# imuncle/TSCM_Calib

Hardware: AMD Instinct MI355X
Metric: LM iterations/sec at 4 cams x 10k views (joint intrinsics+extrinsics, fp64) (higher is better)
Workload: dtype f64; 1 GPU; BASELINE config 4: 4 cams x 10000 views/cam, 20000 frames, 2160000 corners (9x6 board, sigma=0.1 px, seed 20244); parallelism=frames sharded over 1 GPU(s)

## Files before the change

include/tscm/tscm.h:

```cpp
#ifndef TSCM_H
#define TSCM_H

#include <stddef.h>

#ifdef __cplusplus
extern "C" {
#endif

#define TSCM_ABI_VERSION 6

enum {
    TSCM_OK = 0,
    TSCM_E_INVALID = -1,
    TSCM_E_NO_DEVICE = -2,
    TSCM_E_HIP = -3,
    TSCM_E_RCCL = -4,
    TSCM_E_UNSUPPORTED = -5,
    TSCM_E_NOMEM = -6,
    TSCM_E_PEER = -7
};

enum { TSCM_CONVERGENCE = 0, TSCM_NO_CONVERGENCE = 1, TSCM_FAILURE = 2 };

#define TSCM_MAX_ITERATIONS 255
// ... 76 lines not shown
    double seconds_solve;
    double seconds_total;
    double rmse;
} tscm_summary;

typedef struct tscm_solver tscm_solver;
typedef struct tscm_comm tscm_comm;

int tscm_abi_version(void);
const char *tscm_last_error(void);
int tscm_device_count(void);
int tscm_device_synchronize(int device);
int tscm_device_peak_fp64(int device, double *mfma_tflops, double *valu_tflops);
int tscm_device_peak_fp64_ex(int device, double peaks[3]);
int tscm_device_peak_fp32_mfma(int device, double *tflops);

void tscm_default_options(tscm_options *opt, int mono);

int tscm_solver_create(const tscm_problem *problem, int device, tscm_solver **out);
int tscm_solver_set_comm(tscm_solver *s, tscm_comm *comm);
int tscm_solver_debug_withhold_handoff(tscm_solver *s, int on);
int tscm_solver_debug_schur_rot(tscm_solver *s, int rot);
int tscm_solver_debug_reduced_backsub(tscm_solver *s, int on);
int tscm_solver_reruns(const tscm_solver *s);
int tscm_solver_solve(tscm_solver *s, const tscm_options *opt, tscm_summary *summary);
int tscm_solver_upload_params(tscm_solver *s, const double *cam_rt, const double *intr, const double *board_rt);
int tscm_solver_solve_resident(tscm_solver *s, const tscm_options *opt, tscm_summary *summary, int reset);
int tscm_solver_download_params(tscm_solver *s, double *cam_rt, double *intr, double *board_rt);
void tscm_solver_destroy(tscm_solver *s);
int tscm_solver_kernel_time(tscm_solver *s, int enable, int *launches, double *total_ms);
int tscm_solver_exchange_time(tscm_solver *s, int *n_T, double *ms_T, int *n_H, double *ms_H);

int tscm_solve_multi(const tscm_problem *problem, const tscm_options *opt, tscm_summary *summary);
int tscm_solve_mono(const tscm_problem *problem, const tscm_options *opt, tscm_summary *summary);

int tscm_eval_functor(const tscm_problem *problem, int device, double *residuals,
                      double *J_cam, double *J_board, double *J_intr, double *cost);

int tscm_eval_normal_equations(const tscm_problem *problem, int device, double *board_gram,
                               double *board_grad, double *view_cross, double *cam_gram,
                               double *cam_grad, double *cost);

int tscm_eval_normal_equations_ex(const tscm_problem *problem, int device, const tscm_options *opt,
                                  double *board_gram, double *board_grad, double *view_cross,
                                  double *cam_gram, double *cam_grad, double *cost);

// ... 540 lines not shown
```

tscm_calib_amd/api.py:

```python
from __future__ import annotations

import ctypes as C

import numpy as np

from . import lib as _l
from .problem import Problem


class Solver:

    def __init__(self, problem: Problem, device: int = 0, rank: int = 0, world: int = 1, *, weights=None, priors=None):
        self.problem = problem.normalised() if not _is_normalised(problem) else problem
        self.problem.validate()
        self._built, w = _l.corner_weights(self.problem, weights)
        self._cp = _l.c_problem(self._built)
        self._h = C.c_void_p()
        self.rank, self.world = rank, world
        _l.check(_l.lib().tscm_solver_create_sharded(C.byref(self._cp), device, rank, world, C.byref(self._h)))
        self._comm = None
        if w is not None:
            _l.check(_l.lib().tscm_solver_set_corner_weights(self._h, _l.dptr(w)))
        if priors is not None:
            self.set_camera_priors(priors)
# ... 23 lines not shown
        if weights is None:
            _l.check(_l.lib().tscm_solver_set_corner_weights(self._h, None))
            return
        _, w = _l.corner_weights(self.problem, weights, self._built.view_count)
        _l.check(_l.lib().tscm_solver_set_corner_weights(self._h, _l.dptr(w)))

    def set_fixed_intrinsics(self, fixed):
        w = _l.fixed_masks(fixed, self.problem.n_cameras)
        _l.check(_l.lib().tscm_solver_set_fixed_intrinsics(self._h, _l.ushort_ptr(w)))

    def set_camera_priors(self, priors):
        ptr, keep = _l.priors_ptr(priors, self.problem.n_cameras)
        _l.check(_l.lib().tscm_solver_set_camera_priors(self._h, ptr))
        del keep

    def debug_withhold_handoff(self, on=True):
        _l.check(_l.lib().tscm_solver_debug_withhold_handoff(self._h, int(on)))

    def debug_schur_rot(self, rot=0):
        _l.check(_l.lib().tscm_solver_debug_schur_rot(self._h, int(rot)))

    def debug_reduced_backsub(self, on=True):
        _l.check(_l.lib().tscm_solver_debug_reduced_backsub(self._h, int(bool(on))))

    def reruns(self) -> int:
        n = _l.lib().tscm_solver_reruns(self._h)
        if n < 0:
            _l.check(n)
        return n

    def solve(self, **options) -> dict:
        o = _l.default_options(self.problem.mono, **options)
        s = _l.CSummary()
        _l.check(_l.lib().tscm_solver_solve(self._h, C.byref(o), C.byref(s)))
        return _l.summary_dict(s)

    def upload_params(self, cam_rt=None, intr=None, board_rt=None):
        p = self.problem
        cam_rt = p.cam_rt if cam_rt is None else np.ascontiguousarray(cam_rt, dtype=np.float64)
        intr = p.intr if intr is None else np.ascontiguousarray(intr, dtype=np.float64)
        board_rt = p.board_rt if board_rt is None else np.ascontiguousarray(board_rt, dtype=np.float64)
        _l.check(_l.lib().tscm_solver_upload_params(self._h, _l.dptr(cam_rt), _l.dptr(intr), _l.dptr(board_rt)))

    def solve_resident(self, reset: bool = True, **options) -> dict:
        o = _l.default_options(self.problem.mono, **options)
        s = _l.CSummary()
# ... 109 lines not shown
    def solve_resident(self, reset: bool = True, **options) -> "list[dict]":
        o = _l.default_options(self.problem.mono, **options)
        hs = (C.c_void_p * self.world)(*[s._h for s in self.solvers])
        sums = (_l.CSummary * self.world)()
        _l.check(_l.lib().tscm_solver_solve_group(hs, self.world, C.byref(o), sums, 1 if reset else 0))
        return [_l.summary_dict(sums[r]) for r in range(self.world)]

    def close(self):
        for s in self.solvers:
            s.close()
        for c in self.comms:
            c.close()
        self.solvers, self.comms = [], []

    def __enter__(self):
        return self

    def __exit__(self, *a):
        self.close()


def debug_reduced_backsub_default(on=True):
    _l.check(_l.lib().tscm_solver_debug_reduced_backsub(None, int(bool(on))))


def _is_normalised(p: Problem) -> bool:
    ok = lambda a, dt: isinstance(a, np.ndarray) and a.dtype == dt and a.flags["C_CONTIGUOUS"]
    return (all(ok(getattr(p, n), np.float64) for n in ("board_xy", "obs_u", "obs_v", "cam_rt", "intr", "board_rt"))
            and all(ok(getattr(p, n), np.int32) for n in ("view_camera", "view_board", "view_offset", "view_count"))
            and ok(p.cam_pose_constant, np.uint8)
            and (p.board_pose_constant is None or ok(p.board_pose_constant, np.uint8)))


def camera_priors(problem: Problem, intr_sigma=None, cam_rt_sigma=None, mean=None, pixel_sigma: float = 1.0) -> "_l.CameraPriors":
    Cn = problem.n_cameras
    mean = mean or {}

    def weights(sig, per):
        s = np.broadcast_to(np.asarray(sig, dtype=np.float64), (Cn, per)).copy()
        if np.any(s < 0.0):
            raise ValueError("a prior's sigma must not be negative")
        w = np.zeros((Cn, per))
        ok = np.isfinite(s) & (s > 0.0)
        w[ok] = (float(pixel_sigma) / s[ok]) ** 2
        return w

# ... 488 lines not shown
```

tscm_calib_amd/csrc/tscm_columns.h:

```cpp
#ifndef TSCM_COLUMNS_H
#define TSCM_COLUMNS_H

#include "tscm_layout.h"
#include "tscm_nd_plan.h"
#include "tscm_exec_plan.h"

#include <algorithm>
#include <string>
#include <utility>
#include <vector>

namespace tscm {

constexpr int kColFree = 13;
constexpr int kColGrad = 13;

struct SolveTile { bool mine, rhsrow; int ri, cj; };
template <int TS, int G>
inline SolveTile solve_tile(int tid, int NP)
{
    constexpr int NT = (G * G + 63) / 64 * 64;
    auto owns = [&](int t) { const int ti = t / G, tj = t % G; return tj <= ti && ti < NP; };
    SolveTile t;
    t.mine = owns(tid); t.rhsrow = false;
// ... 10 lines not shown
constexpr int kMapOne = 1 << 30;
constexpr int kSolveMapThreads = 256;

constexpr int kExtNone = 0, kExtRow = 3, kExtSol = 4;
constexpr int kSolveExtPanels = 12;
TSCM_LAYOUT_FN bool solve_tile_live(int kind, int ri, int cj, int from, int tk)
{
    if (kind == kExtNone || !(ri > tk && cj >= tk && tk >= from)) return false;
    if (ri == cj && ri == tk + 1) return false;
    return !(kind == kExtRow && cj == tk);
}

struct ColumnPlan {
    std::vector<unsigned char> col_active;
    std::vector<unsigned char> col_ctl;
    std::vector<int> act_map;
    int n_act = 0;
    int cam_pre[9] = {};
    unsigned short cam_free[8] = {};
    std::vector<Int4> solve_map;
    std::vector<Int4> solve_ext;
    bool ext_fallback = false;
    int wave_sum_old = 0, wave_sum_new = 0;
    bool has_nd = false;
    NdPlan nd[2];
};

inline std::vector<Int4> plan_solve_map(const Layout &L, const ColumnPlan &c)
{
    constexpr int TS = 4, G = 16, NT = kSolveMapThreads;
    static_assert(NT == (G * G + 63) / 64 * 64, "one map entry per thread of k_solve_reduced<4, 16>");
    const int NP = (c.n_act + TS - 1) / TS;
    auto cmap = [&](int ci) { return ci < c.n_act ? c.act_map[ci] : -1; };
    auto t_offset = [&](int i, int j) {
        int lo = i >> 4, hi = j >> 4, a = i & 15, b = j & 15;
        if (lo > hi) { std::swap(lo, hi); std::swap(a, b); }
        const int bit = lo * 8 + hi;
        const unsigned long long m = L.pair_mask;
        return ((m >> bit) & 1ull) ? 256 * __builtin_popcountll(m & ((1ull << bit) - 1ull)) + a * 16 + b : -1;
    };
    std::vector<Int4> map((size_t)(kSolveMapSlots / 4) * NT);
    for (int tid = 0; tid < NT; ++tid) {
        const SolveTile tl = solve_tile<TS, G>(tid, NP);
        int off[kSolveMapSlots];
        std::fill(off, off + kSolveMapSlots, -1);
        off[kMapTile] = tl.ri; off[kMapTile + 1] = tl.cj; off[kMapTile + 2] = tl.mine ? 1 : tl.rhsrow ? 2 : 0;
// ... 46 lines not shown
    for (int i = 0; i < NP; ++i) {
        for (int j = i; j < NP; ++j) tiles.push_back(Tile{ kExtRow, NP + 1 + i, j, i, i, j - 1 });
        tiles.push_back(Tile{ kExtSol, NP + 1 + i, NP, i, i, NP - 1 });
    }
    std::stable_sort(tiles.begin(), tiles.end(), [](const Tile &a, const Tile &b) { return a.last != b.last ? a.last > b.last : a.first < b.first; });
    size_t room = 0;
    for (const auto &f : free_tid) room += f.size();
    if (room < tiles.size()) { c.ext_fallback = true; return; }
    std::vector<size_t> used(NW, 0);
    for (const Tile &t : tiles) {
        int best = -1, best_add = 0, best_base = 0;
        for (int w = 0; w < NW - 1; ++w) {
            if (used[w] == free_tid[w].size()) continue;
            int add = 0, base = 0;
            for (int tk = 0; tk < NP; ++tk) { add += tk >= t.first && tk <= t.last && !live[w][tk]; base += live[w][tk]; }
            if (best < 0 || add < best_add || (add == best_add && base > best_base)) { best = w; best_add = add; best_base = base; }
        }
        c.solve_ext[(size_t)free_tid[best][used[best]++]] = Int4{ t.kind, t.ri, t.cj, t.i };
        for (int tk = t.first; tk <= t.last; ++tk) live[best][tk] = 1;
    }
    c.wave_sum_new = wave_sum();
}

inline int plan_columns(const Layout &L, int C, const unsigned short *fixed, ColumnPlan &out, std::string &err)
{
    ColumnPlan c;
    const int n_pad = 16 * C;
    c.col_active.assign((size_t)n_pad, 0); c.col_ctl.assign((size_t)16 * kMaxCam, 0);
    std::vector<unsigned short> word(C, 0);
    for (int i = 0; i < n_pad; ++i) {
        const int m = i >> 4, a = i & 15;
        const bool act = L.cam_active[m] != 0, cst = L.cam_const[m] != 0;
        const unsigned f = fixed ? fixed[m] : 0u;
        const bool held = a >= 6 && a < kColFree && ((f >> (a - 6)) & 1u);
        const bool block_const = (f & TSCM_FIX_INTRINSICS) == TSCM_FIX_INTRINSICS;
        c.col_active[i] = (a < kColFree && act && !(a < 6 && cst) && !held) ? 1 : 0;
        const bool in_x = a < 6 ? (act && !cst) : a < 15 ? (act && !block_const) : false;
        c.col_ctl[i] = (unsigned char)((in_x ? 1 : 0) | (c.col_active[i] ? 2 : 0));
        if (c.col_active[i]) word[m] |= (unsigned short)(1u << a);
    }
    c.act_map.assign((size_t)n_pad, -1);
    for (int i = 0; i < n_pad; ++i) if (c.col_active[i]) c.act_map[c.n_act++] = i;
    std::fill(c.cam_pre, c.cam_pre + 9, c.n_act);
    if (C <= kMaxCamLds) {
        int run = 0;
        for (int m = 0; m < C; ++m) { c.cam_pre[m] = run; c.cam_free[m] = word[m]; run += __builtin_popcount(word[m]); }
    }
    if (C <= kDense4Cams) { c.solve_map = plan_solve_map(L, c); plan_solve_ext(c); }
    if (C <= kMaxCamLds && c.n_act > 0) {
        int ncols[kMaxCamLds];
        std::vector<int> cols((size_t)16 * C, -1);
        for (int m = 0; m < C; ++m) {
            ncols[m] = 0;
            for (int a = 0; a < 16; ++a) if ((word[m] >> a) & 1u) cols[16 * (size_t)m + ncols[m]++] = 16 * m + a;
        }
        if (!nd_build_plans_cols(C, ncols, cols.data(), L.pair_present.data(), L.bid_of.data(), c.nd))
            return layout_fail(err, TSCM_E_UNSUPPORTED, "internal error: the reduced system does not fit the register/LDS solver");
        const std::vector<int> want(c.act_map.begin(), c.act_map.begin() + c.n_act);
        for (const NdPlan &pl : c.nd) {
            std::vector<int> pc;
            for (int col : pl.pcol) if (col >= 0) pc.push_back(col);
            std::sort(pc.begin(), pc.end());
            if (pc != want) return layout_fail(err, TSCM_E_UNSUPPORTED, "internal error: elimination plan does not cover the free columns");
        }
        c.has_nd = true;
    }
    out = std::move(c);
    return 0;
}

}
// ... 3 lines not shown
```

tscm_calib_amd/csrc/tscm_solve_dense4.h:

```cpp
#pragma once

__device__ __forceinline__ double load_T_small(const DevProblem &P, const double *T, int i, int j)
{
    int lo = i >> 4, hi = j >> 4, a = i & 15, b = j & 15;
    if (lo > hi) { const int t = lo; lo = hi; hi = t; const int u = a; a = b; b = u; }
    const int bit = lo * 8 + hi;
    const unsigned long long m = P.pair_mask;
    const int tile = __popcll(m & ((1ull << bit) - 1ull));
    return ((m >> bit) & 1ull) ? T[256 * tile + a * 16 + b] : 0.0;
}

__host__ __device__ __forceinline__ int kth_set_bit16(unsigned w, int k)
{
    int pos = 0, c;
    c = __builtin_popcount(w & 0xffu); if (k >= c) { k -= c; w >>= 8; pos += 8; }
    c = __builtin_popcount(w & 0xfu);  if (k >= c) { k -= c; w >>= 4; pos += 4; }
    c = __builtin_popcount(w & 0x3u);  if (k >= c) { k -= c; w >>= 2; pos += 2; }
    c = (int)(w & 1u);                 if (k >= c) pos += 1;
    return pos;
}
__device__ __forceinline__ int compact_to_padded(const DevProblem &P, int ci)
{
    int base = 0, q0 = 0;
    unsigned w = P.cam_free[0];
// ... 182 lines not shown
        }
    };
    auto load_tile = [&](const double *src, double (&t)[TS][TS]) {
#pragma unroll
        for (int r = 0; r < TS; ++r)
#pragma unroll
            for (int c = 0; c < TS; ++c) t[r][c] = src[r * TS + c];
    };
    auto panel_solve = [&](const double (&At)[TS][TS], const PanelFactor &f, double (&x)[TS][TS]) {
#pragma unroll
        for (int r = 0; r < TS; ++r)
#pragma unroll
            for (int c = 0; c < TS; ++c) {
                double v = At[r][c];
#pragma unroll
                for (int q = 0; q < c; ++q) v -= x[r][q] * f.l[c][q];
                x[r][c] = v * f.il[c];
            }
    };
    __shared__ __attribute__((aligned(16))) double s_dt[2][TS * TS];
    const bool dthread = tid == NT - 1;
    if (cj == 0 && ri > 0 && pub) publish_tile(lds + xo, a);
    if (ri == 1 && cj == 1 && mine) publish_tile(s_dt[0], a);
    if (tid == 0 && NP > 0) factor_diag(a, 0);
    __syncthreads();
    for (int tk = 0; tk < NP; ++tk) {
        const double *Ar = Xb + (tk & 1) * (G * XT);
#ifdef TSCM_PHASE_PROFILE
        __shared__ long long s_ph[8];
        if (tk == 3 && (dthread || tid == 11 * G + 5)) s_ph[dthread ? 0 : 4] = wall_clock64();
#endif
        if (dthread && tk + 1 < NP) {
            PanelFactor f;
            double araw[TS][TS], dt[TS][TS], x[TS][TS], t[TS][TS];
            load_factor(f, tk);
            load_tile(Ar + (tk + 1) * XT, araw);
            load_tile(s_dt[tk & 1], dt);
            __builtin_amdgcn_sched_barrier(0);
            panel_solve(araw, f, x);
#pragma unroll
            for (int r = 0; r < TS; ++r)
#pragma unroll
                for (int c = 0; c <= r; ++c) {
                    double v = dt[r][c];
#pragma unroll
                    for (int q = 0; q < TS; ++q) v -= x[r][q] * x[c][q];
                    t[r][c] = v;
                }
#ifdef TSCM_PHASE_PROFILE
            if (tk == 3) { asm volatile("" : "+v"(t[3][3])); s_ph[1] = wall_clock64(); }
#endif
            factor_diag(t, tk + 1);
#ifdef TSCM_PHASE_PROFILE
// ... 16 lines not shown
                if (rhsrow) {
#pragma unroll
                    for (int c = 0; c < TS; ++c) wp[tk * TS + c] = xi[0][c];
                }
            } else {
                double xj[TS][TS];
                panel_solve(aj, f, xj);
#pragma unroll
                for (int r = 0; r < TS; ++r)
#pragma unroll
                    for (int c = 0; c < TS; ++c) {
                        double v = a[r][c];
#pragma unroll
                        for (int q = 0; q < TS; ++q) v -= xi[r][q] * xj[c][q];
                        a[r][c] = v;
                    }
            }
        }
        {
            const bool col = cj == tk + 1 && ri > tk + 1 && pub, dg = ri == tk + 2 && cj == tk + 2 && mine;
            if (col || dg) publish_tile(col ? lds + xo + ((tk + 1) & 1) * xs : s_dt[(tk + 1) & 1], a);
        }
#ifdef TSCM_PHASE_PROFILE
        if (tk == 3 && tid == 11 * G + 5) { asm volatile("" : "+v"(a[3][3])); s_ph[5] = wall_clock64(); }
        if (tk + 1 < NP) __syncthreads();
        if (tk == 3 && tid == 0) { s_ph[6] = wall_clock64(); printf("  panel 3: D x,t %lld  factor %lld | update %lld | to barrier exit %lld\n", s_ph[1] - s_ph[0], s_ph[2] - s_ph[1], s_ph[5] - s_ph[4], s_ph[6] - s_ph[0]); }
#else
        if (tk + 1 < NP) __syncthreads();
#endif
    }
    if (stile) {
#pragma unroll
        for (int r = 0; r < TS; ++r) { const int pc = s_c2p[from * TS + r]; if (pc >= 0) yv[pc] = -a[r][0]; }
    }
    if (!ext_on && cj < ri && mine) {
#pragma unroll
        for (int r = 0; r < TS; ++r)
#pragma unroll
            for (int c = 0; c < TS; ++c) Lm[(ri * TS + r) * LD + cj * TS + c] = a[r][c];
    }
    __syncthreads();
    PHASE_STAMP(ts2);
#ifdef TSCM_PHASE_PROFILE
    const long long cy2 = clock64();
#endif
    TailOperands tail_ops = {};
    if (!ext_on) tail_prefetch(P, S, cur, H, tail_ops);
// ... 54 lines not shown
```

tscm_calib_amd/csrc/tscm_solver.hip:

```cpp
#include "tscm/tscm.h"
#include "tscm_host.h"
#include "tscm_kernels.h"
#include "tscm_launch_seq.h"
#include "tscm_mono_batch.h"

#include <hip/hip_runtime.h>
#include <hip/hip_ext.h>
#include <rccl/rccl.h>

#include <algorithm>
#include <atomic>
#include <chrono>
#include <cstdio>
#include <cstdlib>
#include <cmath>
#include <cstring>
#include <memory>
#include <numeric>
#include <string>
#include <thread>
#include <vector>

using namespace tscm;

// ... 95 lines not shown
    NdPlan plan[2];
    const int4 *d_nd_map[2] = { nullptr, nullptr };
    const int *d_nd_tab[2] = { nullptr, nullptr }, *d_nd_bs[2] = { nullptr, nullptr };
    size_t lds_nd[2] = { 0, 0 }, lds_dense4 = 0;
    size_t lds_eval4 = 0;
    EvalKernel eval[kEvalFamilies] = {};
    LossArg loss{};
    bool weighted = false;
    double *d_obs_w = nullptr;
    std::vector<double> h_obs_u, h_obs_v;
    std::vector<int> p_view_count;
    double w_sum = 0.0;
    long n_kept = 0;
    std::vector<double> pr_cam_mean, pr_cam_w, pr_intr_mean, pr_intr_w;
    std::vector<unsigned char> col_free;
    double *d_prior = nullptr;
    int n_priors = 0;
    PriorArg prior_arg() const { return PriorArg{ d_prior, d_prior + 16 * (size_t)C }; }
    std::vector<unsigned short> fixed;
    int n_cu = 1;
    int schur_rot = 0;
    bool ext_planned = false;
    bool force_backsub = false;
    double *d_view_sq = nullptr;
    int timing = 0;
    unsigned ev_count[3] = { 0, 0, 0 };
    std::vector<std::pair<hipEvent_t, hipEvent_t>> ev;
    std::vector<int> ev_kind;
    size_t ev_used = 0;
    int t_launches[3] = { 0, 0, 0 };
    double t_ms[3] = { 0.0, 0.0, 0.0 };
};

struct SolverDelete { void operator()(tscm_solver *s) const { tscm_solver_destroy(s); } };
using SolverPtr = std::unique_ptr<tscm_solver, SolverDelete>;

static int create_scoped(const tscm_problem *p, int device, SolverPtr &sp)
{
    tscm_solver *s = nullptr;
    if (int rc = tscm_solver_create(p, device, &s)) return rc;
    sp.reset(s);
    return 0;
}

extern "C" int tscm_abi_version(void) { return TSCM_ABI_VERSION; }
extern "C" const char *tscm_last_error(void) { return g_err.c_str(); }
// ... 124 lines not shown
{
    if (!s) return fail(TSCM_E_INVALID, "solver is NULL");
    if (int rc = check_camera_priors(priors, s->C)) return rc;
    if (priors && s->world > 1) return fail(TSCM_E_UNSUPPORTED, "camera priors on a sharded solver (world > 1) are not supported");
    auto keep = [&](std::vector<double> &dst, const double *src, int per) { if (priors && src) dst.assign(src, src + per * (size_t)s->C); else dst.clear(); };
    keep(s->pr_cam_mean, priors ? priors->cam_rt_mean : nullptr, 6); keep(s->pr_cam_w, priors ? priors->cam_rt_weight : nullptr, 6);
    keep(s->pr_intr_mean, priors ? priors->intr_mean : nullptr, 9); keep(s->pr_intr_w, priors ? priors->intr_weight : nullptr, 9);
    return refresh_priors(s);
}

extern "C" void tscm_solver_destroy(tscm_solver *s)
{
    if (!s) return;
    (void)hipSetDevice(s->device);
    s->stream = s->own_stream;
    if (s->stream) (void)hipStreamSynchronize(s->stream);
    for (auto &e : s->ev) { (void)hipEventDestroy(e.first); (void)hipEventDestroy(e.second); }
    if (s->h_ctrl) (void)hipHostFree(s->h_ctrl);
    if (s->stream) (void)hipStreamDestroy(s->stream);
    delete s;
}

static std::atomic<bool> g_force_backsub{ false };

static int apply_columns(tscm_solver *s, const ColumnPlan &c)
{
    DevProblem &P = s->P;
    HIP_TRY(hipSetDevice(s->device));
    HIP_TRY(hipStreamSynchronize(s->stream));
    HIP_TRY(hipMemcpy(const_cast<unsigned char *>(P.col_active), c.col_active.data(), c.col_active.size(), hipMemcpyHostToDevice));
    HIP_TRY(hipMemcpy(const_cast<unsigned char *>(P.col_ctl), c.col_ctl.data(), c.col_ctl.size(), hipMemcpyHostToDevice));
    HIP_TRY(hipMemcpy(const_cast<int *>(P.act_map), c.act_map.data(), sizeof(int) * c.act_map.size(), hipMemcpyHostToDevice));
    P.n_act = c.n_act;
    std::copy(std::begin(c.cam_pre), std::end(c.cam_pre), P.cam_pre);
    std::copy(std::begin(c.cam_free), std::end(c.cam_free), P.cam_free);
    static_assert(sizeof(Int4) == sizeof(int4), "the operand map is uploaded as it is");
    if (!c.solve_map.empty()) {
        HIP_TRY(hipMemcpy(const_cast<int4 *>(P.solve_map), c.solve_map.data(), sizeof(Int4) * c.solve_map.size(), hipMemcpyHostToDevice));
        HIP_TRY(hipMemcpy(const_cast<int4 *>(P.solve_ext), c.solve_ext.data(), sizeof(Int4) * c.solve_ext.size(), hipMemcpyHostToDevice));
        s->ext_planned = !c.ext_fallback;
        P.solve_ext_on = s->ext_planned && !s->force_backsub;
    }
    if (c.has_nd) {
        for (int v = 0; v < 2; ++v) {
            const NdPlan &pl = c.nd[v];
            s->mem.release(s->d_nd_map[v]); s->mem.release(s->d_nd_tab[v]); s->mem.release(s->d_nd_bs[v]);
            s->d_nd_map[v] = nullptr; s->d_nd_tab[v] = nullptr; s->d_nd_bs[v] = nullptr;
            HIP_TRY(s->mem.upload(&s->d_nd_map[v], reinterpret_cast<const int4 *>(pl.map.data()), pl.map.size() / 4));
            HIP_TRY(s->mem.upload(&s->d_nd_tab[v], pl.tab));
            HIP_TRY(s->mem.upload(&s->d_nd_bs[v], pl.bs_tab));
            s->lds_nd[v] = sizeof(double) * pl.lds_doubles;
            s->plan[v] = pl;
        }
        {
            const size_t lds_max = std::max(std::max(s->lds_nd[0], s->lds_nd[1]), s->lds_bs);
            if (lds_max > 64 * 1024)
                for (const void *k : { reinterpret_cast<const void *>(k_solve_nd<1, true>), reinterpret_cast<const void *>(k_solve_nd<2, true>),
                                       reinterpret_cast<const void *>(k_solve_nd<1, false>), reinterpret_cast<const void *>(k_solve_nd<2, false>) })
                    HIP_TRY(hipFuncSetAttribute(k, hipFuncAttributeMaxDynamicSharedMemorySize, (int)lds_max));
        }
        for (int v = 0; v < 2; ++v) {
            const size_t lds = std::max(s->lds_nd[v], s->lds_bs);
            int per_cu = 0;
            if (s->plan[v].tpt == 1) HIP_TRY(hipOccupancyMaxActiveBlocksPerMultiprocessor(&per_cu, reinterpret_cast<const void *>(k_solve_nd<1, true>), kNdThreads, lds));
// ... 149 lines not shown
    for (int *flag : { S.t_count, S.y_flag, S.fac_fail }) HIP_TRY(hipMemset(flag, 0, sizeof(int)));
    for (int k = 0; k < 2; ++k) if (V) HIP_TRY(hipMemset(S.rec[k], 0, sizeof(double) * (size_t)kRec * V));
    HIP_TRY(hipMemset(S.stats_count, 0, 256)); HIP_TRY(hipMemset(S.stats_flag, 0, 256));
    HIP_TRY(hipMemset(S.ctl_pub, 0, sizeof(CtlPub)));
    HIP_TRY(hipMemset(S.T, 0, sizeof(double) * 256 * (size_t)L.n_bids));
    HIP_TRY(hipMemset(S.H_stage, 0, sizeof(double) * (256 * (size_t)C + kScal + world)));
    HIP_TRY(hipMemset(S.campart2, 0, sizeof(double) * 512 * (size_t)C));
    HIP_TRY(hipMemset(S.ctrl, 0, sizeof(Ctrl)));
    HIP_TRY(hipMemset(S.ctrl_snap, 0, sizeof(CtrlHead)));
    HIP_TRY(hipHostMalloc(reinterpret_cast<void **>(&s->h_ctrl), sizeof(Ctrl)));
    HIP_TRY(hipHostGetDevicePointer(reinterpret_cast<void **>(&s->d_h_ctrl), s->h_ctrl, 0));

    s->lds_eval = 4 * lds_eval_bytes;
    s->lds_eval32 = sizeof(double) * (size_t)eval_f32_lds_doubles(p->n_points, g4.ks);
    s->lds_eval4 = lds_eval4;
    if (s->lds_eval32 > 64 * 1024)
        for (int f = F32; f < kEvalFamilies; ++f) HIP_TRY(hipFuncSetAttribute(reinterpret_cast<const void *>(s->eval[f]), hipFuncAttributeMaxDynamicSharedMemorySize, (int)s->lds_eval32));
    ColumnPlan cols;
    {
        std::string err;
        if (int rc = plan_columns(L, C, nullptr, cols, err)) return fail(rc, err);
    }
    if (C <= kDense4Cams) {
        int4 *map = nullptr;
        HIP_TRY(s->mem.alloc(&map, (size_t)(kSolveMapSlots / 4) * kSolveMapThreads));
        P.solve_map = map;
        int4 *ext = nullptr;
        HIP_TRY(s->mem.alloc(&ext, (size_t)kSolveMapThreads));
        P.solve_ext = ext;
        s->force_backsub = g_force_backsub.load();
        const size_t NN = 64, TT = 4, NPD = 64;
        s->lds_dense4 = sizeof(double) * (NN * (NN + 2) + 2 * (NN / TT) * (TT * TT + 2) + 2 * NN + 3 * NPD);
        int per_cu = 0;
        HIP_TRY(hipOccupancyMaxActiveBlocksPerMultiprocessor(&per_cu, reinterpret_cast<const void *>(k_solve_reduced<4, 16, 64, true>), 256, std::max(s->lds_dense4, s->lds_bs)));
        s->dev.dense4_resident = per_cu * prop.multiProcessorCount;
    }
    if (C > kMaxCamLds) {
        const int NN = (cols.n_act + 15) & ~15;
        const size_t lds_max = solve_big_lds_bytes(NN, s->n_pad);
        HIP_TRY(s->mem.alloc(&S.Abig, (size_t)256 * (NN / 16 + 1) * (NN / 16 + 2) / 2));
        if (lds_max > 64 * 1024) HIP_TRY(hipFuncSetAttribute(reinterpret_cast<const void *>(k_solve_reduced_big), hipFuncAttributeMaxDynamicSharedMemorySize, (int)lds_max));
    }
    if (int rc = apply_columns(s, cols)) return rc;
    if (s->lds_eval > 160 * 1024) return fail(TSCM_E_UNSUPPORTED, "board has too many corners for the LDS board-point tile");
    HIP_TRY(hipDeviceSynchronize());
    *out = sp.release();
    return 0;
}

extern "C" int tscm_solver_create(const tscm_problem *p, int device, tscm_solver **out)
{
    return tscm_solver_create_sharded(p, device, 0, 1, out);
}
// ... 1 lines not shown
static CommKind comm_kind(const tscm_comm *c) { return !c ? kCommNone : c->world > 1 || c->group ? kCommShared : kCommOneRank; }

extern "C" int tscm_solver_debug_withhold_handoff(tscm_solver *s, int on)
{
    if (!s) return fail(TSCM_E_INVALID, "solver is NULL");
    s->withhold_next = on == 3 ? kWithholdStats : on ? kWithholdProducer : 0;
    s->no_rerun_next = on == 2;
    return 0;
}

extern "C" int tscm_solver_debug_schur_rot(tscm_solver *s, int rot)
{
    if (!s) return fail(TSCM_E_INVALID, "solver is NULL");
    if (rot != 0 && rot != 2) return fail(TSCM_E_INVALID, "rot must be 0 or 2");
    s->schur_rot = rot;
    return 0;
}

extern "C" int tscm_solver_debug_reduced_backsub(tscm_solver *s, int on)
{
    if (on != 0 && on != 1) return fail(TSCM_E_INVALID, "on must be 0 or 1");
    if (!s) { g_force_backsub.store(on != 0); return 0; }
    s->force_backsub = on != 0;
    s->P.solve_ext_on = s->ext_planned && !s->force_backsub;
    return 0;
}

extern "C" int tscm_solver_reruns(const tscm_solver *s)
{
    if (!s) return fail(TSCM_E_INVALID, "solver is NULL");
    return s->n_reruns;
}

extern "C" int tscm_solver_set_comm(tscm_solver *s, tscm_comm *comm)
{
    if (!s) return fail(TSCM_E_INVALID, "solver is NULL");
    if (comm && comm->device != s->device) return fail(TSCM_E_INVALID, "communicator and solver live on different devices");
    if (comm && (comm->world != s->world || comm->rank != s->rank))
        return fail(TSCM_E_INVALID, "communicator rank / world differ from the solver's shard (tscm_solver_create_sharded)");
    s->comm_reg = comm;
    s->comm = uses_comm(comm_kind(comm), 0) ? comm : nullptr;
    return 0;
}

extern "C" int tscm_solver_upload_params(tscm_solver *s, const double *cam_rt, const double *intr, const double *board_rt)
{
    if (!s || !intr || (!board_rt && s->L.B_total)) return fail(TSCM_E_INVALID, "NULL argument");
// ... 191 lines not shown
    }
    double *buf = t_buffer ? s0->S.T : s0->S.H_stage;
    if (int rc = timed_begin(s0, t_buffer ? 1 : 2, s0->stream, &e1)) return rc;
    if (int rc = comm_allreduce(s0->comm, buf, n, s0->stream)) return rc;
    if (e1) HIP_TRY(hipEventRecord(e1, s0->stream));
    return 0;
}

static int enqueue(tscm_solver *s, const Launch &l)
{
    const DevProblem &P = s->P;
    const DevState &S = s->S;
    hipStream_t st = s->stream;
    const dim3 grid(l.grid);
    auto schur = [&](auto kernel) { hipLaunchKernelGGL(kernel, grid, dim3(256), 0, st, P, S, l.chunk0, l.ctl, l.first_round, l.ce, l.target, l.n_chunks, s->schur_rot); };
    auto nd = [&](auto kernel) {
        const int v = l.nd;
        hipLaunchKernelGGL(kernel, grid, dim3(kNdThreads), std::max(s->lds_nd[v], l.n_bs ? s->lds_bs : (size_t)0), st, P, S, s->d_nd_map[v], s->d_nd_tab[v], s->d_nd_bs[v],
                           s->plan[v].dims(), l.epoch, l.withhold, l.n_prod, l.n_bs, l.f32);
    };
    const size_t lds_dense4 = std::max(s->lds_dense4, l.n_bs ? s->lds_bs : (size_t)0);
    auto dense4 = [&](auto kernel) {
        DevProblem Pd = P;
        if (s->xp.f32()) Pd.solve_ext_on = 0;
        hipLaunchKernelGGL(kernel, grid, dim3(256), lds_dense4, st, Pd, S, l.epoch, l.withhold, l.n_prod, l.n_bs, l.f32);
    };
    switch (l.k) {
    case Kern::BeginViewPrep: {
        const bool init = l.start == Start::Init, bak = l.start == Start::Backup;
        hipLaunchKernelGGL(k_begin_view_prep, grid, dim3(kVPrepThreads), 0, st, P, S, s->head,
                           init ? s->d_init_cam : bak ? s->d_start_cam : nullptr, init ? s->d_init_intr : bak ? s->d_start_intr : nullptr,
                           init ? s->d_init_board : bak ? s->d_start_board : nullptr,
                           bak ? nullptr : s->d_start_cam, bak ? nullptr : s->d_start_intr, bak ? nullptr : s->d_start_board, l.f32);
        break;
    }
    case Kern::Eval: return launch_eval(s, l.cand);
    case Kern::ReduceControl: hipLaunchKernelGGL(k_reduce_control, grid, dim3(256), 0, st, P, S, l.cand, l.init, l.have_backsub); break;
    case Kern::ReduceStats:
        if (s->xp.priors) hipLaunchKernelGGL(k_reduce_stats_prior, grid, dim3(256), 0, st, P, S, l.cand, l.init, s->prior_arg());
        else hipLaunchKernelGGL(k_reduce_stats, grid, dim3(256), 0, st, P, S, l.cand, l.init);
        break;
    case Kern::FinalizeEval: hipLaunchKernelGGL(k_finalize_eval, grid, dim3(256), 0, st, P, S, l.have_backsub); break;
    case Kern::Control: hipLaunchKernelGGL(k_control, grid, dim3(256), 0, st, P, S, l.init); break;
    case Kern::SchurFactor: hipLaunchKernelGGL(k_schur_factor, grid, dim3(256), 0, st, P, S); break;
    case Kern::Schur1: schur(k_schur_gram<1>); break;
    case Kern::Schur2: schur(k_schur_gram<2>); break;
    case Kern::Schur3: schur(k_schur_gram<3>); break;
// ... 1104 lines not shown
```

tscm_calib_amd/lib.py:

```python
from __future__ import annotations

import ctypes as C
import os
import subprocess

import numpy as np

_HERE = os.path.dirname(os.path.abspath(__file__))
CSRC = os.path.join(_HERE, "csrc")
LIB_PATH = os.path.join(CSRC, "libtscm_hip.so")
UNIQUE_ID_BYTES = 128
IPC_HANDLE_BYTES = 80
MAX_ITERATIONS = 255
EXEC_SEPARATE_T_REDUCE = 1
EXEC_KEEP_SINGLE_RANK_COMM = 2
EXEC_GRAM_16X16 = 4
EXEC_SEPARATE_BACKSUB = 8
EXEC_SEPARATE_CONTROL = 16
EXEC_DENSE_REDUCED_ORDER = 32
EXEC_GRAPH_REDUCED_ORDER = 64
EXEC_SEPARATE_STATS = 128
LOSS_NONE, LOSS_HUBER, LOSS_SOFT_L1, LOSS_CAUCHY = 0, 1, 2, 3
LOSS_KINDS = {None: LOSS_NONE, "none": LOSS_NONE, "huber": LOSS_HUBER, "soft_l1": LOSS_SOFT_L1, "cauchy": LOSS_CAUCHY}
PROJ_PERSPECTIVE, PROJ_LONGLAT, PROJ_CYLINDRICAL, PROJ_STEREOGRAPHIC, PROJ_EQUIRECT = 0, 1, 2, 3, 4
# ... 153 lines not shown
    _fields_ = [("camera_a", C.c_int), ("camera_b", C.c_int), ("board_rt", C.c_double * 6)]


class CResidualParams(C.Structure):
    _fields_ = [("struct_size", C.c_int), ("loss_kind", C.c_int), ("loss_scale", C.c_double), ("grid_w", C.c_int), ("grid_h", C.c_int),
                ("image_width", C.c_int), ("image_height", C.c_int), ("n_angle_bins", C.c_int), ("pad", C.c_int), ("max_angle", C.c_double),
                ("clamp", C.c_double)]


class CResidualInfo(C.Structure):
    _fields_ = [("struct_size", C.c_int), ("n_views_used", C.c_int), ("n_used", C.c_longlong), ("sum_w", C.c_double), ("cost", C.c_double),
                ("rmse", C.c_double), ("grid_outside", C.c_longlong * 32), ("angle_outside", C.c_longlong * 32), ("seconds_kernel", C.c_double * 4)]


class CCornerSet(C.Structure):
    _fields_ = [
        ("n_cameras", C.c_int), ("n_boards", C.c_int), ("board_cols", C.c_int), ("board_rows", C.c_int), ("pitch", C.c_double),
        ("image_width", C.c_int), ("image_height", C.c_int), ("has", C.c_void_p), ("pix_u", C.c_void_p), ("pix_v", C.c_void_p),
    ]


EXPORTS = [
    "tscm_abi_version", "tscm_last_error", "tscm_device_count", "tscm_device_synchronize", "tscm_device_peak_fp64", "tscm_device_peak_fp64_ex", "tscm_device_peak_fp32_mfma", "tscm_default_options",
    "tscm_solver_create", "tscm_solver_set_comm", "tscm_solver_debug_withhold_handoff", "tscm_solver_debug_schur_rot", "tscm_solver_debug_reduced_backsub", "tscm_solver_reruns", "tscm_solver_solve", "tscm_solver_upload_params",
    "tscm_solver_solve_resident", "tscm_solver_download_params", "tscm_solver_destroy",
    "tscm_solver_kernel_time", "tscm_solver_exchange_time", "tscm_solve_multi", "tscm_solve_mono", "tscm_eval_functor",
    "tscm_eval_normal_equations", "tscm_eval_normal_equations_ex", "tscm_eval_step_ex", "tscm_project_points", "tscm_unproject_pixels",
    "tscm_reprojection_error", "tscm_comm_unique_id", "tscm_comm_create", "tscm_comm_destroy",
    "tscm_shard_frames", "tscm_solver_create_sharded", "tscm_comm_create_local", "tscm_comm_ipc_open", "tscm_comm_ipc_connect", "tscm_solver_solve_group",
    "tscm_solver_gather_boards", "tscm_comm_info", "tscm_rig_init", "tscm_rig_stage_errors", "tscm_yaml_format", "tscm_yaml_write", "tscm_yaml_parse",
    "tscm_yaml_read", "tscm_build_maps", "tscm_estimate_focal", "tscm_poses_from_r1r2t",
    "tscm_estimate_extrinsic", "tscm_estimate_focal_rows", "tscm_estimate_extrinsic_stages", "tscm_corners_write", "tscm_corners_read", "tscm_corners_free",
    "tscm_detect_corners", "tscm_detect_corners_batch", "tscm_corner_planes_batch", "tscm_corner_candidates_free", "tscm_chessboards_from_corners", "tscm_chessboards_free", "tscm_remap",
    "tscm_solver_set_loss", "tscm_solve_robust", "tscm_eval_normal_equations_robust", "tscm_eval_step_robust",
    "tscm_solver_eval_normal_equations",
    "tscm_solver_set_fixed_intrinsics", "tscm_solve_fixed", "tscm_eval_step_fixed", "tscm_solve_mono_batch",
    "tscm_covariance", "tscm_covariance_from_normal_equations",
    "tscm_solver_set_corner_weights", "tscm_solve_weighted", "tscm_eval_normal_equations_weighted", "tscm_eval_step_weighted",
    "tscm_solve_mono_batch_weighted", "tscm_covariance_weighted",
    "tscm_solver_set_camera_priors", "tscm_solve_prior", "tscm_eval_normal_equations_prior", "tscm_eval_step_prior", "tscm_covariance_prior",
    "tscm_projection_uncertainty", "tscm_projection_uncertainty_seconds",
    "tscm_view_gain", "tscm_view_gain_apply", "tscm_view_gain_seconds",
    "tscm_residual_default_params", "tscm_residual_report", "tscm_residual_debug_chunk_target",
    "tscm_build_maps_ex", "tscm_rectify_points",
    "tscm_stereo_default_params", "tscm_stereo_match", "tscm_stereo_stages", "tscm_stereo_stage_times", "tscm_stereo_points",
    "tscm_stereo_filter_default_params", "tscm_stereo_filter", "tscm_stereo_filter_stages",
    "tscm_stereo_fill_default_params", "tscm_stereo_fill", "tscm_stereo_fill_stages",
# ... 30 lines not shown
    L = C.CDLL(LIB_PATH)
    dp, ip, vp = C.POINTER(C.c_double), C.POINTER(C.c_int), C.c_void_p
    L.tscm_abi_version.restype = C.c_int
    L.tscm_last_error.restype = C.c_char_p
    L.tscm_device_count.restype = C.c_int
    L.tscm_device_synchronize.argtypes = [C.c_int]
    L.tscm_device_peak_fp64.argtypes = [C.c_int, dp, dp]
    L.tscm_device_peak_fp64_ex.argtypes = [C.c_int, dp]
    L.tscm_device_peak_fp32_mfma.argtypes = [C.c_int, dp]
    L.tscm_default_options.argtypes = [C.POINTER(COptions), C.c_int]
    L.tscm_default_options.restype = None
    L.tscm_solver_create.argtypes = [C.POINTER(CProblem), C.c_int, C.POINTER(vp)]
    L.tscm_solver_create_sharded.argtypes = [C.POINTER(CProblem), C.c_int, C.c_int, C.c_int, C.POINTER(vp)]
    L.tscm_comm_create_local.argtypes = [C.c_int, C.c_int, C.POINTER(vp)]
    L.tscm_comm_ipc_open.argtypes = [C.c_int, C.c_int, C.c_int, C.c_size_t, C.POINTER(vp), C.POINTER(C.c_ubyte)]
    L.tscm_comm_ipc_connect.argtypes = [vp, C.POINTER(C.c_ubyte)]
    L.tscm_solver_solve_group.argtypes = [C.POINTER(vp), C.c_int, C.POINTER(COptions), C.POINTER(CSummary), C.c_int]
    L.tscm_solver_gather_boards.argtypes = [vp, dp]
    L.tscm_comm_info.argtypes = [vp, ip, ip, ip]
    L.tscm_solver_set_comm.argtypes = [vp, vp]
    L.tscm_solver_debug_withhold_handoff.argtypes = [vp, C.c_int]
    L.tscm_solver_debug_schur_rot.argtypes = [vp, C.c_int]
    L.tscm_solver_debug_reduced_backsub.argtypes = [vp, C.c_int]
    L.tscm_solver_reruns.argtypes = [vp]
    L.tscm_solver_solve.argtypes = [vp, C.POINTER(COptions), C.POINTER(CSummary)]
    L.tscm_solver_upload_params.argtypes = [vp, dp, dp, dp]
    L.tscm_solver_solve_resident.argtypes = [vp, C.POINTER(COptions), C.POINTER(CSummary), C.c_int]
    L.tscm_solver_download_params.argtypes = [vp, dp, dp, dp]
    L.tscm_solver_destroy.argtypes = [vp]
    L.tscm_solver_destroy.restype = None
    L.tscm_solver_kernel_time.argtypes = [vp, C.c_int, ip, dp]
    L.tscm_solver_exchange_time.argtypes = [vp, ip, dp, ip, dp]
    L.tscm_solve_multi.argtypes = [C.POINTER(CProblem), C.POINTER(COptions), C.POINTER(CSummary)]
    L.tscm_solve_mono.argtypes = [C.POINTER(CProblem), C.POINTER(COptions), C.POINTER(CSummary)]
    L.tscm_eval_functor.argtypes = [C.POINTER(CProblem), C.c_int, dp, dp, dp, dp, dp]
    L.tscm_eval_normal_equations.argtypes = [C.POINTER(CProblem), C.c_int, dp, dp, dp, dp, dp, dp]
    L.tscm_eval_normal_equations_ex.argtypes = [C.POINTER(CProblem), C.c_int, C.POINTER(COptions), dp, dp, dp, dp, dp, dp]
    L.tscm_eval_step_ex.argtypes = [C.POINTER(CProblem), C.c_int, C.POINTER(COptions), dp, dp, dp, ip, C.POINTER(CSummary)]
    L.tscm_solver_set_loss.argtypes = [vp, C.c_int, C.c_double]
    L.tscm_solve_robust.argtypes = [C.POINTER(CProblem), C.POINTER(COptions), C.c_int, C.c_double, C.POINTER(CSummary)]
    L.tscm_eval_normal_equations_robust.argtypes = [C.POINTER(CProblem), C.c_int, C.POINTER(COptions), C.c_int, C.c_double, dp, dp, dp, dp, dp, dp]
    L.tscm_eval_step_robust.argtypes = [C.POINTER(CProblem), C.c_int, C.POINTER(COptions), C.c_int, C.c_double, dp, dp, dp, ip, C.POINTER(CSummary)]
    L.tscm_solver_eval_normal_equations.argtypes = [vp, C.POINTER(COptions), C.c_int, dp, dp, dp, dp, dp, dp]
    usp = C.POINTER(C.c_ushort)
    L.tscm_solver_set_fixed_intrinsics.argtypes = [vp, usp]
    L.tscm_solve_fixed.argtypes = [C.POINTER(CProblem), C.POINTER(COptions), usp, C.c_int, C.c_double, C.POINTER(CSummary)]
# ... 309 lines not shown
```

Before: 9469 LM iterations/s.

## Reseat dense Schur solve tiles onto threads to retire waves early

Adds a host-side planner that permutes which thread owns each tile in the dense 4-camera Schur factorization. Tiles are grouped into wavefronts by the last panel in which they are live, so whole waves go idle sooner. The remapped operand tables are uploaded in two variants, one for the extended path and one for backsub or f32. The kernel now picks the diagonal-factor thread by tile ownership instead of thread id 0. The plan is kept only when it lowers the count of active waves summed over panels, and it adds extra device tables plus a debug toggle.

```diff
diff --git a/include/tscm/tscm.h b/include/tscm/tscm.h
--- a/include/tscm/tscm.h
+++ b/include/tscm/tscm.h
@@ -122,6 +122,8 @@
 int tscm_solver_debug_withhold_handoff(tscm_solver *s, int on);
 int tscm_solver_debug_schur_rot(tscm_solver *s, int rot);
 int tscm_solver_debug_reduced_backsub(tscm_solver *s, int on);
+int tscm_solver_debug_solve_seating(tscm_solver *s, int on);
+int tscm_solver_solve_seating_info(const tscm_solver *s, int *info);
 int tscm_solver_reruns(const tscm_solver *s);
 int tscm_solver_solve(tscm_solver *s, const tscm_options *opt, tscm_summary *summary);
 int tscm_solver_upload_params(tscm_solver *s, const double *cam_rt, const double *intr, const double *board_rt);
diff --git a/tscm_calib_amd/api.py b/tscm_calib_amd/api.py
--- a/tscm_calib_amd/api.py
+++ b/tscm_calib_amd/api.py
@@ -69,6 +69,14 @@
 
     def debug_reduced_backsub(self, on=True):
         _l.check(_l.lib().tscm_solver_debug_reduced_backsub(self._h, int(bool(on))))
+
+    def debug_solve_seating(self, on=True):
+        _l.check(_l.lib().tscm_solver_debug_solve_seating(self._h, int(bool(on))))
+
+    def solve_seating_info(self) -> dict:
+        info = (C.c_int * 4)()
+        _l.check(_l.lib().tscm_solver_solve_seating_info(self._h, info))
+        return dict(zip(("moved", "wave_sum_new", "wave_sum_seated", "wave_sum_seated_backsub"), (int(v) for v in info)))
 
     def reruns(self) -> int:
         n = _l.lib().tscm_solver_reruns(self._h)
@@ -224,6 +232,10 @@
 
 def debug_reduced_backsub_default(on=True):
     _l.check(_l.lib().tscm_solver_debug_reduced_backsub(None, int(bool(on))))
+
+
+def debug_solve_seating_default(on=True):
+    _l.check(_l.lib().tscm_solver_debug_solve_seating(None, int(bool(on))))
 
 
 def _is_normalised(p: Problem) -> bool:
diff --git a/tscm_calib_amd/csrc/tscm_columns.h b/tscm_calib_amd/csrc/tscm_columns.h
--- a/tscm_calib_amd/csrc/tscm_columns.h
+++ b/tscm_calib_amd/csrc/tscm_columns.h
@@ -56,6 +56,10 @@
     std::vector<Int4> solve_ext;
     bool ext_fallback = false;
     int wave_sum_old = 0, wave_sum_new = 0;
+    std::vector<int> solve_seat;
+    int wave_sum_seated = 0;
+    std::vector<int> solve_seat_backsub;
+    int wave_sum_seated_backsub = 0;
     bool has_nd = false;
     NdPlan nd[2];
 };
@@ -148,6 +152,63 @@
     c.wave_sum_new = wave_sum();
 }
 
+inline int solve_seat_wave_sum(const ColumnPlan &c, const std::vector<int> &seat, bool ext_on, std::vector<int> *per_panel = nullptr)
+{
+    constexpr int TS = 4, NT = kSolveMapThreads, NW = NT / 64;
+    const int NP = (c.n_act + TS - 1) / TS;
+    std::vector<int> waves((size_t)std::max(NP, 1), 0);
+    int sum = 0;
+    for (int tk = 0; tk < NP; ++tk) {
+        bool any[NW] = {};
+        for (int t = 0; t < NT; ++t) {
+            const Int4 m = c.solve_map[(size_t)(kMapTile / 4) * NT + t], e = ext_on ? c.solve_ext[t] : Int4{ kExtNone, 0, 0, 0 };
+            if (e.x ? solve_tile_live(e.x, e.y, e.z, e.w, tk) : solve_tile_live(m.z, m.x, m.y, 0, tk)) any[seat[t] / 64] = true;
+        }
+        for (int w = 0; w < NW; ++w) { waves[tk] += any[w]; sum += any[w]; }
+    }
+    if (per_panel) *per_panel = waves;
+    return sum;
+}
+
+inline int seat_solve_tiles(const ColumnPlan &c, bool ext_on, int pinned_sum, std::vector<int> &seat_out)
+{
+    constexpr int TS = 4, NT = kSolveMapThreads, NS = NT - 64;
+    const int NP = (c.n_act + TS - 1) / TS;
+    seat_out.resize((size_t)NT);
+    for (int t = 0; t < NT; ++t) seat_out[t] = t;
+    int last[NS], order[NS];
+    for (int t = 0; t < NS; ++t) {
+        const Int4 m = c.solve_map[(size_t)(kMapTile / 4) * NT + t], e = ext_on ? c.solve_ext[t] : Int4{ kExtNone, 0, 0, 0 };
+        last[t] = -1; order[t] = t;
+        for (int tk = 0; tk < NP; ++tk) if (e.x ? solve_tile_live(e.x, e.y, e.z, e.w, tk) : solve_tile_live(m.z, m.x, m.y, 0, tk)) last[t] = tk;
+    }
+    std::stable_sort(order, order + NS, [&](int a, int b) { return last[a] > last[b]; });
+    std::vector<int> seat(seat_out);
+    for (int w = 0; w < NS / 64; ++w) {
+        int *o = order + 64 * w;
+        std::sort(o, o + 64);
+        for (int l = 0; l < 64; ++l) seat[o[l]] = NS - 64 * (w + 1) + l;
+    }
+    const int sum = solve_seat_wave_sum(c, seat, ext_on);
+    if (sum >= pinned_sum) return pinned_sum;
+    seat_out = seat;
+    return sum;
+}
+inline void plan_solve_seat(ColumnPlan &c)
+{
+    c.wave_sum_seated = seat_solve_tiles(c, !c.ext_fallback, c.wave_sum_new, c.solve_seat);
+    c.wave_sum_seated_backsub = seat_solve_tiles(c, false, c.wave_sum_old, c.solve_seat_backsub);
+}
+
+inline std::vector<Int4> seated_table(const std::vector<Int4> &logical, const std::vector<int> &seat)
+{
+    constexpr int NT = kSolveMapThreads;
+    std::vector<Int4> out(logical.size());
+    for (size_t q = 0; q < logical.size() / NT; ++q)
+        for (int t = 0; t < NT; ++t) out[q * NT + seat[t]] = logical[q * NT + t];
+    return out;
+}
+
 inline int plan_columns(const Layout &L, int C, const unsigned short *fixed, ColumnPlan &out, std::string &err)
 {
     ColumnPlan c;
@@ -172,7 +233,7 @@
         int run = 0;
         for (int m = 0; m < C; ++m) { c.cam_pre[m] = run; c.cam_free[m] = word[m]; run += __builtin_popcount(word[m]); }
     }
-    if (C <= kDense4Cams) { c.solve_map = plan_solve_map(L, c); plan_solve_ext(c); }
+    if (C <= kDense4Cams) { c.solve_map = plan_solve_map(L, c); plan_solve_ext(c); plan_solve_seat(c); }
     if (C <= kMaxCamLds && c.n_act > 0) {
         int ncols[kMaxCamLds];
         std::vector<int> cols((size_t)16 * C, -1);
diff --git a/tscm_calib_amd/csrc/tscm_solve_dense4.h b/tscm_calib_amd/csrc/tscm_solve_dense4.h
--- a/tscm_calib_amd/csrc/tscm_solve_dense4.h
+++ b/tscm_calib_amd/csrc/tscm_solve_dense4.h
@@ -228,13 +228,13 @@
     const bool dthread = tid == NT - 1;
     if (cj == 0 && ri > 0 && pub) publish_tile(lds + xo, a);
     if (ri == 1 && cj == 1 && mine) publish_tile(s_dt[0], a);
-    if (tid == 0 && NP > 0) factor_diag(a, 0);
+    if (mine && ri == 0 && cj == 0) factor_diag(a, 0);
     __syncthreads();
     for (int tk = 0; tk < NP; ++tk) {
         const double *Ar = Xb + (tk & 1) * (G * XT);
 #ifdef TSCM_PHASE_PROFILE
         __shared__ long long s_ph[8];
-        if (tk == 3 && (dthread || tid == 11 * G + 5)) s_ph[dthread ? 0 : 4] = wall_clock64();
+        if (tk == 3 && (dthread || (mine && ri == 11 && cj == 5))) s_ph[dthread ? 0 : 4] = wall_clock64();
 #endif
         if (dthread && tk + 1 < NP) {
             PanelFactor f;
@@ -297,7 +297,7 @@
             if (col || dg) publish_tile(col ? lds + xo + ((tk + 1) & 1) * xs : s_dt[(tk + 1) & 1], a);
         }
 #ifdef TSCM_PHASE_PROFILE
-        if (tk == 3 && tid == 11 * G + 5) { asm volatile("" : "+v"(a[3][3])); s_ph[5] = wall_clock64(); }
+        if (tk == 3 && mine && ri == 11 && cj == 5) { asm volatile("" : "+v"(a[3][3])); s_ph[5] = wall_clock64(); }
         if (tk + 1 < NP) __syncthreads();
         if (tk == 3 && tid == 0) { s_ph[6] = wall_clock64(); printf("  panel 3: D x,t %lld  factor %lld | update %lld | to barrier exit %lld\n", s_ph[1] - s_ph[0], s_ph[2] - s_ph[1], s_ph[5] - s_ph[4], s_ph[6] - s_ph[0]); }
 #else
diff --git a/tscm_calib_amd/csrc/tscm_solver.hip b/tscm_calib_amd/csrc/tscm_solver.hip
--- a/tscm_calib_amd/csrc/tscm_solver.hip
+++ b/tscm_calib_amd/csrc/tscm_solver.hip
@@ -141,6 +141,11 @@
     int schur_rot = 0;
     bool ext_planned = false;
     bool force_backsub = false;
+    std::vector<Int4> solve_map, solve_ext;
+    std::vector<int> solve_seat[2];
+    int seat_sums[3] = { 0, 0, 0 };
+    int4 *d_solve_map[2] = { nullptr, nullptr }, *d_solve_ext = nullptr;
+    bool seating = true;
     double *d_view_sq = nullptr;
     int timing = 0;
     unsigned ev_count[3] = { 0, 0, 0 };
@@ -311,6 +316,26 @@
 }
 
 static std::atomic<bool> g_force_backsub{ false };
+static std::atomic<bool> g_seating{ true };
+
+static void select_solve_path(tscm_solver *s)
+{
+    s->P.solve_ext_on = s->ext_planned && !s->force_backsub;
+    s->P.solve_map = s->d_solve_map[s->P.solve_ext_on ? 0 : 1];
+}
+
+static int upload_solve_tables(tscm_solver *s)
+{
+    std::vector<int> ident((size_t)kSolveMapThreads);
+    for (int t = 0; t < kSolveMapThreads; ++t) ident[t] = t;
+    for (int v = 0; v < 2; ++v) {
+        const std::vector<Int4> map = seated_table(s->solve_map, s->seating ? s->solve_seat[v] : ident);
+        HIP_TRY(hipMemcpy(s->d_solve_map[v], map.data(), sizeof(Int4) * map.size(), hipMemcpyHostToDevice));
+    }
+    const std::vector<Int4> ext = seated_table(s->solve_ext, s->seating ? s->solve_seat[0] : ident);
+    HIP_TRY(hipMemcpy(s->d_solve_ext, ext.data(), sizeof(Int4) * ext.size(), hipMemcpyHostToDevice));
+    return 0;
+}
 
 static int apply_columns(tscm_solver *s, const ColumnPlan &c)
 {
@@ -325,10 +350,12 @@
     std::copy(std::begin(c.cam_free), std::end(c.cam_free), P.cam_free);
     static_assert(sizeof(Int4) == sizeof(int4), "the operand map is uploaded as it is");
     if (!c.solve_map.empty()) {
-        HIP_TRY(hipMemcpy(const_cast<int4 *>(P.solve_map), c.solve_map.data(), sizeof(Int4) * c.solve_map.size(), hipMemcpyHostToDevice));
-        HIP_TRY(hipMemcpy(const_cast<int4 *>(P.solve_ext), c.solve_ext.data(), sizeof(Int4) * c.solve_ext.size(), hipMemcpyHostToDevice));
+        s->solve_map = c.solve_map; s->solve_ext = c.solve_ext;
+        s->solve_seat[0] = c.solve_seat; s->solve_seat[1] = c.solve_seat_backsub;
+        s->seat_sums[0] = c.wave_sum_new; s->seat_sums[1] = c.wave_sum_seated; s->seat_sums[2] = c.wave_sum_seated_backsub;
+        if (int rc = upload_solve_tables(s)) return rc;
         s->ext_planned = !c.ext_fallback;
-        P.solve_ext_on = s->ext_planned && !s->force_backsub;
+        select_solve_path(s);
     }
     if (c.has_nd) {
         for (int v = 0; v < 2; ++v) {
@@ -524,13 +551,12 @@
         if (int rc = plan_columns(L, C, nullptr, cols, err)) return fail(rc, err);
     }
     if (C <= kDense4Cams) {
-        int4 *map = nullptr;
-        HIP_TRY(s->mem.alloc(&map, (size_t)(kSolveMapSlots / 4) * kSolveMapThreads));
-        P.solve_map = map;
-        int4 *ext = nullptr;
-        HIP_TRY(s->mem.alloc(&ext, (size_t)kSolveMapThreads));
-        P.solve_ext = ext;
+        for (int v = 0; v < 2; ++v) HIP_TRY(s->mem.alloc(&s->d_solve_map[v], (size_t)(kSolveMapSlots / 4) * kSolveMapThreads));
+        HIP_TRY(s->mem.alloc(&s->d_solve_ext, (size_t)kSolveMapThreads));
+        P.solve_map = s->d_solve_map[0];
+        P.solve_ext = s->d_solve_ext;
         s->force_backsub = g_force_backsub.load();
+        s->seating = g_seating.load();
         const size_t NN = 64, TT = 4, NPD = 64;
         s->lds_dense4 = sizeof(double) * (NN * (NN + 2) + 2 * (NN / TT) * (TT * TT + 2) + 2 * NN + 3 * NPD);
         int per_cu = 0;
@@ -578,7 +604,29 @@
     if (on != 0 && on != 1) return fail(TSCM_E_INVALID, "on must be 0 or 1");
     if (!s) { g_force_backsub.store(on != 0); return 0; }
     s->force_backsub = on != 0;
-    s->P.solve_ext_on = s->ext_planned && !s->force_backsub;
+    if (s->d_solve_ext) select_solve_path(s);
+    return 0;
+}
+
+extern "C" int tscm_solver_debug_solve_seating(tscm_solver *s, int on)
+{
+    if (on != 0 && on != 1) return fail(TSCM_E_INVALID, "on must be 0 or 1");
+    if (!s) { g_seating.store(on != 0); return 0; }
+    s->seating = on != 0;
+    if (!s->d_solve_ext) return 0;
+    HIP_TRY(hipSetDevice(s->device));
+    HIP_TRY(hipStreamSynchronize(s->stream));
+    return upload_solve_tables(s);
+}
+
+extern "C" int tscm_solver_solve_seating_info(const tscm_solver *s, int *info)
+{
+    if (!s || !info) return fail(TSCM_E_INVALID, "solver or info is NULL");
+    std::fill(info, info + 4, 0);
+    if (!s->d_solve_ext) return 0;
+    int moved = 0;
+    for (int v = 0; v < 2; ++v) for (int t = 0; t < kSolveMapThreads; ++t) moved += s->seating && s->solve_seat[v][t] != t;
+    info[0] = moved; info[1] = s->seat_sums[0]; info[2] = s->seat_sums[1]; info[3] = s->seat_sums[2];
     return 0;
 }
 
@@ -816,7 +864,7 @@
     const size_t lds_dense4 = std::max(s->lds_dense4, l.n_bs ? s->lds_bs : (size_t)0);
     auto dense4 = [&](auto kernel) {
         DevProblem Pd = P;
-        if (s->xp.f32()) Pd.solve_ext_on = 0;
+        if (s->xp.f32()) { Pd.solve_ext_on = 0; Pd.solve_map = s->d_solve_map[1]; }
         hipLaunchKernelGGL(kernel, grid, dim3(256), lds_dense4, st, Pd, S, l.epoch, l.withhold, l.n_prod, l.n_bs, l.f32);
     };
     switch (l.k) {
diff --git a/tscm_calib_amd/lib.py b/tscm_calib_amd/lib.py
--- a/tscm_calib_amd/lib.py
+++ b/tscm_calib_amd/lib.py
@@ -199,7 +199,7 @@
 
 EXPORTS = [
     "tscm_abi_version", "tscm_last_error", "tscm_device_count", "tscm_device_synchronize", "tscm_device_peak_fp64", "tscm_device_peak_fp64_ex", "tscm_device_peak_fp32_mfma", "tscm_default_options",
-    "tscm_solver_create", "tscm_solver_set_comm", "tscm_solver_debug_withhold_handoff", "tscm_solver_debug_schur_rot", "tscm_solver_debug_reduced_backsub", "tscm_solver_reruns", "tscm_solver_solve", "tscm_solver_upload_params",
+    "tscm_solver_create", "tscm_solver_set_comm", "tscm_solver_debug_withhold_handoff", "tscm_solver_debug_schur_rot", "tscm_solver_debug_reduced_backsub", "tscm_solver_debug_solve_seating", "tscm_solver_solve_seating_info", "tscm_solver_reruns", "tscm_solver_solve", "tscm_solver_upload_params",
     "tscm_solver_solve_resident", "tscm_solver_download_params", "tscm_solver_destroy",
     "tscm_solver_kernel_time", "tscm_solver_exchange_time", "tscm_solve_multi", "tscm_solve_mono", "tscm_eval_functor",
     "tscm_eval_normal_equations", "tscm_eval_normal_equations_ex", "tscm_eval_step_ex", "tscm_project_points", "tscm_unproject_pixels",
@@ -276,6 +276,8 @@
     L.tscm_solver_debug_withhold_handoff.argtypes = [vp, C.c_int]
     L.tscm_solver_debug_schur_rot.argtypes = [vp, C.c_int]
     L.tscm_solver_debug_reduced_backsub.argtypes = [vp, C.c_int]
+    L.tscm_solver_debug_solve_seating.argtypes = [vp, C.c_int]
+    L.tscm_solver_solve_seating_info.argtypes = [vp, ip]
     L.tscm_solver_reruns.argtypes = [vp]
     L.tscm_solver_solve.argtypes = [vp, C.POINTER(COptions), C.POINTER(CSummary)]
     L.tscm_solver_upload_params.argtypes = [vp, dp, dp, dp]
```

After: 9524 LM iterations/s, median of 6. No clear change (+0.6%).
